# Quantus-Network/qp-zk-circuits

Hardware: AMD Instinct MI355X
Metric: Wormhole proofs/sec (higher is better)
Workload: dtype u64

## Files before the change

### include/qpgpu.h

```cpp
#ifndef QPGPU_H
#define QPGPU_H
#include <stddef.h>
#include <stdint.h>

#ifdef __cplusplus
extern "C" {
#endif

typedef struct qpgpu_ctx qpgpu_ctx;
typedef struct qpgpu_circuit qpgpu_circuit;

enum {
    QPGPU_OK = 0,
    QPGPU_EINVAL = -1,
    QPGPU_EDEVICE = -2,
    QPGPU_ENOMEM = -3,
    QPGPU_EUNSAT = -4,
    QPGPU_EBUFSIZE = -5
};

int qpgpu_ctx_create(int device, qpgpu_ctx **out);
void qpgpu_ctx_destroy(qpgpu_ctx *ctx);
const char *qpgpu_last_error(const qpgpu_ctx *ctx);
int qpgpu_ctx_set_stream(qpgpu_ctx *ctx, void *hip_stream);
// ... 20 lines not shown
int qpgpu_set_hasher(int kind, const uint64_t *params, size_t n_words);
int qpgpu_get_hasher(void);

enum {
    QPGPU_NTT_FORWARD = 0,
    QPGPU_NTT_INVERSE = 1,
    QPGPU_NTT_OUT_BITREV = 2
};
int qpgpu_ntt_batch(qpgpu_ctx *ctx, uint64_t *data, unsigned log_n, size_t batch, int flags,
                    uint64_t coset_shift);
int qpgpu_ntt_batch_dev(qpgpu_ctx *ctx, const uint64_t *d_in, uint64_t *d_out, unsigned log_n,
                        size_t batch, int flags, uint64_t coset_shift);
int qpgpu_lde_batch_dev(qpgpu_ctx *ctx, const uint64_t *d_coeffs, uint64_t *d_out, unsigned log_n,
                        unsigned rate_bits, size_t batch, int flags, uint64_t coset_shift);

int qpgpu_poseidon_permute_dev(qpgpu_ctx *ctx, uint64_t *d_states, size_t n);
int qpgpu_poseidon2_hash_pad10_dev(qpgpu_ctx *ctx, const uint64_t *params, size_t n_words, const uint64_t *d_in, size_t len,
                                   size_t count, uint64_t *d_out);
size_t qpgpu_merkle_digest_count(unsigned log_leaves, unsigned cap_height);
int qpgpu_merkle_build_dev(qpgpu_ctx *ctx, const uint64_t *d_cols, uint64_t col_stride, uint32_t n_cols,
                           unsigned log_leaves, unsigned cap_height, uint64_t *d_digests, uint64_t *h_cap_out);
int qpgpu_merkle_build_rows_dev(qpgpu_ctx *ctx, const uint64_t *d_rows, uint32_t width, unsigned log_leaves,
                                unsigned cap_height, uint64_t *d_digests, uint64_t *h_cap_out);

int qpgpu_circuit_load(qpgpu_ctx *ctx, const uint64_t *pack_words, size_t n_words, qpgpu_circuit **out);
int qpgpu_circuit_load_batch(qpgpu_ctx *ctx, const uint64_t *pack_words, size_t n_words, unsigned max_batch, qpgpu_circuit **out);
unsigned qpgpu_circuit_max_batch(const qpgpu_circuit *c);
size_t qpgpu_circuit_num_public_inputs(const qpgpu_circuit *c);
void qpgpu_circuit_free(qpgpu_circuit *c);
int qpgpu_circuit_scrub(qpgpu_circuit *c);
int qpgpu_circuit_constants_sigmas_cap(const qpgpu_circuit *c, uint64_t *out, size_t out_words);
int qpgpu_circuit_set_blinding_seed(qpgpu_circuit *c, uint64_t seed);
int qpgpu_circuit_set_witness_check(qpgpu_circuit *c, int on);
size_t qpgpu_proof_size(const qpgpu_circuit *c);
int qpgpu_prove(qpgpu_circuit *c, const uint64_t *wires, const uint64_t *public_inputs, uint8_t *out, size_t out_cap, size_t *out_len);
int qpgpu_prove_dev(qpgpu_circuit *c, const uint64_t *d_wires, const uint64_t *public_inputs, uint8_t *out, size_t out_cap, size_t *out_len);
int qpgpu_prove_batch_dev(qpgpu_circuit *c, const uint64_t *const *d_wires, uint32_t batch, const uint64_t *const *public_inputs,
                          uint8_t *const *outs, size_t out_cap, size_t *out_lens);

int qpgpu_witness_info(qpgpu_circuit *c, uint64_t *num_generators, uint64_t *num_levels, uint64_t *num_free_cells);
int qpgpu_witness_free_mask(qpgpu_circuit *c, uint8_t *mask, size_t mask_len);
int qpgpu_generate_witness_dev(qpgpu_circuit *c, uint64_t *d_wires, const uint64_t *public_inputs);
int qpgpu_generate_witness(qpgpu_circuit *c, uint64_t *wires, const uint64_t *public_inputs);
int qpgpu_circuit_gate_rows(const qpgpu_circuit *c, unsigned gate_type, uint32_t *rows_out, size_t cap, size_t *count);
int qpgpu_generate_witness_batch_dev(qpgpu_circuit *c, uint64_t *d_wires, uint32_t batch, const uint64_t *public_inputs);
int qpgpu_generate_witness_partial_dev(qpgpu_circuit *c, const uint64_t *cells, const uint64_t *values, size_t count,
                                       const uint64_t *public_inputs, uint64_t *d_wires);
int qpgpu_generate_witness_partial_batch_dev(qpgpu_circuit *c, const uint64_t *cells, size_t count, const uint64_t *values,
                                             const uint64_t *public_inputs, uint32_t batch, uint64_t *d_wires, int *status);
int qpgpu_witness_partial_prepare(qpgpu_circuit *c, const uint64_t *cells, size_t count, uint32_t max_batch);
int qpgpu_generate_witness_partial_batch_blinded_dev(qpgpu_circuit *c, const uint64_t *cells, size_t count, size_t n_blinding, const uint64_t *values,
                                                     const uint8_t *seeds, const uint64_t *public_inputs, uint32_t batch, uint64_t *d_wires, int *status);
int qpgpu_witness_public_inputs_dev(qpgpu_circuit *c, const uint64_t *d_wires, uint32_t batch, uint64_t *public_inputs_out);

typedef struct qpgpu_oracle qpgpu_oracle;
#define QPGPU_ORACLE_VALUES 0u
#define QPGPU_ORACLE_COEFFS 1u
#define QPGPU_ORACLE_BLINDING 2u
#define QPGPU_ORACLE_DEVICE_INPUT 4u
int qpgpu_oracle_commit(qpgpu_ctx *ctx, const uint64_t *polys, uint32_t num_polys, unsigned degree_bits, unsigned rate_bits,
                        unsigned cap_height, unsigned flags, uint64_t blinding_seed, uint32_t blinding_stream, qpgpu_oracle **out);
void qpgpu_oracle_free(qpgpu_oracle *o);
int qpgpu_oracle_cap(const qpgpu_oracle *o, uint64_t *out, size_t out_words);
int qpgpu_oracle_eval(qpgpu_oracle *o, const uint64_t point[2], uint32_t first, uint32_t count, uint64_t *out);
#define QPGPU_ORACLE_READ_COEFFS 0u
#define QPGPU_ORACLE_READ_LDE 1u
// ... 73 lines not shown
```

### qp-zk-circuits_amd/binding.py

```python
import ctypes
import os

import numpy as np

P = 0xFFFFFFFF00000001
MULT_GEN = 14293326489335486720

NTT_FORWARD = 0
NTT_INVERSE = 1
NTT_OUT_BITREV = 2

_HERE = os.path.dirname(os.path.abspath(__file__))


def lib_path():
    return os.path.join(_HERE, "libqpgpu.so")


class QpGpuError(RuntimeError):
    def __init__(self, code, msg):
        super().__init__(f"qpgpu error {code}: {msg}")
        self.code = code


# ... 44 lines not shown
        "qpgpu_zk_tree_build": (c.c_int, [vp, vp, c.c_size_t, c.c_uint, c.c_uint, c.POINTER(vp), c.c_char_p]),
        "qpgpu_zk_tree_free": (None, [vp]),
        "qpgpu_zk_tree_depth": (c.c_uint, [vp]),
        "qpgpu_zk_tree_leaf_count": (c.c_size_t, [vp]),
        "qpgpu_zk_tree_root": (c.c_int, [vp, vp]),
        "qpgpu_zk_tree_read_level": (c.c_int, [vp, c.c_uint, c.c_size_t, c.c_size_t, vp]),
        "qpgpu_zk_tree_open": (c.c_int, [vp, vp, c.c_size_t, vp, vp]),
        "qpgpu_zk_tree_build_reserved": (c.c_int, [vp, vp, c.c_size_t, c.c_size_t, c.c_uint, c.c_uint, c.POINTER(vp), c.c_char_p]),
        "qpgpu_zk_tree_capacity": (c.c_size_t, [vp]),
        "qpgpu_zk_tree_append": (c.c_int, [vp, vp, c.c_size_t, c.c_uint, vp, c.c_char_p]),
        "qpgpu_zk_tree_snapshot": (c.c_int, [vp, vp]),
        "qpgpu_zk_tree_open_at": (c.c_int, [vp, vp, vp, c.c_size_t, vp, vp]),
        "qpgpu_poseidon2_hash_pad10": (c.c_int, [u64p, c.c_size_t, u64p, c.c_size_t, u64p]),
        "qpgpu_crash_trace_armed": (c.c_int, []),
        "qpgpu_circuit_num_public_inputs": (c.c_size_t, [vp]),
        "qpgpu_merkle_digest_count": (c.c_size_t, [c.c_uint, c.c_uint]),
        "qpgpu_merkle_build_dev": (c.c_int, [vp, u64p, c.c_uint64, c.c_uint32, c.c_uint, c.c_uint, u64p, u64p]),
        "qpgpu_merkle_build_rows_dev": (c.c_int, [vp, u64p, c.c_uint32, c.c_uint, c.c_uint, u64p, u64p]),
        "qpgpu_circuit_load": (c.c_int, [vp, u64p, c.c_size_t, c.POINTER(vp)]),
        "qpgpu_circuit_load_batch": (c.c_int, [vp, u64p, c.c_size_t, c.c_uint, c.POINTER(vp)]),
        "qpgpu_circuit_max_batch": (c.c_uint, [vp]),
        "qpgpu_circuit_scrub": (c.c_int, [vp]),
        "qpgpu_prove_batch_dev": (c.c_int, [vp, vp, c.c_uint32, vp, vp, c.c_size_t, vp]),
        "qpgpu_ctx_set_hasher": (c.c_int, [vp, c.c_int, u64p, c.c_size_t]),
        "qpgpu_ctx_get_hasher": (c.c_int, [vp]),
        "qpgpu_ctx_challenger_observe": (c.c_int, [vp, vp, u64p, c.c_size_t]),
        "qpgpu_ctx_challenger_get": (c.c_int, [vp, vp, c.POINTER(c.c_uint64)]),
        "qpgpu_pool_create_batched": (c.c_int, [c.c_int, u64p, c.c_size_t, c.c_uint, c.c_uint, c.POINTER(vp)]),
        "qpgpu_circuit_free": (None, [vp]),
        "qpgpu_circuit_constants_sigmas_cap": (c.c_int, [vp, u64p, c.c_size_t]),
        "qpgpu_proof_size": (c.c_size_t, [vp]),
        "qpgpu_circuit_set_blinding_seed": (c.c_int, [vp, c.c_uint64]),
        "qpgpu_circuit_set_witness_check": (c.c_int, [vp, c.c_int]),
        "qpgpu_circuit_gate_rows": (c.c_int, [vp, c.c_uint, vp, c.c_size_t, c.POINTER(c.c_size_t)]),
        "qpgpu_prove": (c.c_int, [vp, u64p, u64p, vp, c.c_size_t, c.POINTER(c.c_size_t)]),
        "qpgpu_prove_dev": (c.c_int, [vp, u64p, u64p, vp, c.c_size_t, c.POINTER(c.c_size_t)]),
        "qpgpu_poseidon_constants": (c.c_size_t, [u64p, u64p, c.c_size_t]),
        "qpgpu_pool_create": (c.c_int, [c.c_int, u64p, c.c_size_t, c.c_uint, c.POINTER(vp)]),
        "qpgpu_pool_destroy": (None, [vp]),
        "qpgpu_pool_proof_size": (c.c_size_t, [vp]),
        "qpgpu_pool_workers": (c.c_uint, [vp]),
        "qpgpu_pool_last_error": (c.c_char_p, [vp]),
        "qpgpu_pool_submit": (c.c_int, [vp, u64p, u64p, vp, c.c_size_t, c.POINTER(c.c_uint64)]),
        "qpgpu_pool_wait": (c.c_int, [vp, c.c_uint64, c.POINTER(c.c_size_t)]),
        "qpgpu_pool_set_witness_check": (c.c_int, [vp, c.c_int]),
        "qpgpu_pool_create_multi": (c.c_int, [vp, c.c_uint, u64p, c.c_size_t, c.c_uint, c.c_uint, c.c_uint, c.POINTER(vp)]),
        "qpgpu_pool_devices": (c.c_uint, [vp]),
        "qpgpu_pool_serialized": (c.c_int, [vp]),
        "qpgpu_pool_set_partial_cells": (c.c_int, [vp, u64p, c.c_size_t]),
        "qpgpu_pool_set_partial_cells_blinded": (c.c_int, [vp, u64p, c.c_size_t, c.c_size_t]),
        "qpgpu_pool_submit_on": (c.c_int, [vp, c.c_uint, u64p, u64p, vp, c.c_size_t, c.POINTER(c.c_uint64)]),
        "qpgpu_pool_submit_host": (c.c_int, [vp, u64p, u64p, vp, c.c_size_t, c.POINTER(c.c_uint64)]),
        "qpgpu_pool_submit_partial": (c.c_int, [vp, u64p, u64p, vp, c.c_size_t, c.POINTER(c.c_uint64)]),
        "qpgpu_set_hasher": (c.c_int, [c.c_int, u64p, c.c_size_t]),
        "qpgpu_get_hasher": (c.c_int, []),
        "qpgpu_witness_info": (c.c_int, [vp, c.POINTER(c.c_uint64), c.POINTER(c.c_uint64), c.POINTER(c.c_uint64)]),
        "qpgpu_witness_free_mask": (c.c_int, [vp, vp, c.c_size_t]),
        "qpgpu_generate_witness_dev": (c.c_int, [vp, u64p, u64p]),
        "qpgpu_generate_witness": (c.c_int, [vp, u64p, u64p]),
        "qpgpu_generate_witness_batch_dev": (c.c_int, [vp, u64p, c.c_uint32, u64p]),
        "qpgpu_generate_witness_partial_dev": (c.c_int, [vp, u64p, u64p, c.c_size_t, u64p, u64p]),
        "qpgpu_generate_witness_partial_batch_dev": (c.c_int, [vp, u64p, c.c_size_t, u64p, u64p, c.c_uint32, u64p, vp]),
        "qpgpu_generate_witness_partial_batch_blinded_dev": (c.c_int, [vp, u64p, c.c_size_t, c.c_size_t, u64p, c.c_char_p, u64p, c.c_uint32, u64p, vp]),
        "qpgpu_witness_public_inputs_dev": (c.c_int, [vp, u64p, c.c_uint32, u64p]),
        "qpgpu_witness_partial_prepare": (c.c_int, [vp, u64p, c.c_size_t, c.c_uint32]),
        "qpgpu_oracle_commit": (c.c_int, [vp, u64p, c.c_uint32, c.c_uint, c.c_uint, c.c_uint, c.c_uint, c.c_uint64, c.c_uint32,
# ... 282 lines not shown
        h = ctypes.c_void_p()
        gpu._check(gpu.lib.qpgpu_circuit_load_batch(gpu.ctx, pw.ctypes.data, pw.size, max_batch, ctypes.byref(h)))
        self.h = h
        self.max_batch = max_batch
        self.num_public_inputs = int(pw[9])

    def scrub(self):
        self.gpu._check(self.gpu.lib.qpgpu_circuit_scrub(self.h))

    def prove_batch_dev(self, d_wires_list, public_inputs_list, outs=None):
        nb = len(d_wires_list)
        ptrs = (ctypes.c_void_p * nb)(*[_ptr(w) for w in d_wires_list])
        pis = [np.ascontiguousarray(p, dtype=np.uint64) for p in public_inputs_list]
        pip = (ctypes.c_void_p * nb)(*[p.ctypes.data for p in pis])
        size = self.proof_size()
        if outs is None:
            outs = [np.empty(size, dtype=np.uint8) for _ in range(nb)]
        op = (ctypes.c_void_p * nb)(*[o.ctypes.data for o in outs])
        lens = (ctypes.c_size_t * nb)()
        self.gpu._check(self.gpu.lib.qpgpu_prove_batch_dev(self.h, ptrs, nb, pip, op, size, lens))
        return [outs[i][:lens[i]].tobytes() for i in range(nb)]

    def close(self):
        if self.h:
            self.gpu.lib.qpgpu_circuit_free(self.h)
            self.h = None

    def proof_size(self):
        return self.gpu.lib.qpgpu_proof_size(self.h)

    def set_witness_check(self, on=True):
        self.gpu._check(self.gpu.lib.qpgpu_circuit_set_witness_check(self.h, 1 if on else 0))

    def set_blinding_seed(self, seed):
        self.gpu._check(self.gpu.lib.qpgpu_circuit_set_blinding_seed(self.h, seed))

    def constants_sigmas_cap(self, cap_height=4):
        out = np.empty((1 << cap_height, 4), dtype=np.uint64)
        self.gpu._check(self.gpu.lib.qpgpu_circuit_constants_sigmas_cap(self.h, out.ctypes.data, out.size))
        return out

    def witness_info(self):
        a, b, c3 = ctypes.c_uint64(), ctypes.c_uint64(), ctypes.c_uint64()
        self.gpu._check(self.gpu.lib.qpgpu_witness_info(self.h, ctypes.byref(a), ctypes.byref(b), ctypes.byref(c3)))
        return a.value, b.value, c3.value

    def gate_rows(self, gate_type):
        n = ctypes.c_size_t()
        self.gpu._check(self.gpu.lib.qpgpu_circuit_gate_rows(self.h, gate_type, None, 0, ctypes.byref(n)))
        rows = np.empty(n.value, dtype=np.uint32)
        self.gpu._check(self.gpu.lib.qpgpu_circuit_gate_rows(self.h, gate_type, rows.ctypes.data, rows.size, ctypes.byref(n)))
        return rows

    def witness_free_mask(self, num_wires, n):
        m = np.empty((num_wires, n), dtype=np.uint8)
        self.gpu._check(self.gpu.lib.qpgpu_witness_free_mask(self.h, m.ctypes.data, m.size))
        return m

    def generate_witness(self, wires, public_inputs):
        w = np.array(wires, dtype=np.uint64, order="C", copy=True)
        p = np.ascontiguousarray(public_inputs, dtype=np.uint64)
        self.gpu._check(self.gpu.lib.qpgpu_generate_witness(self.h, w.ctypes.data, p.ctypes.data))
        return w

    def generate_witness_dev(self, d_wires, public_inputs, batch=1):
        p = np.ascontiguousarray(public_inputs, dtype=np.uint64)
# ... 464 lines not shown
```

### qp-zk-circuits_amd/csrc/circuit_state.hpp

```cpp
#pragma once
#include <hip/hip_runtime.h>
#include <algorithm>
#include <vector>
#include "circuit.hpp"
#include "ctx.hpp"
#include "prover_host.hpp"
#include "prover_kernels.hpp"

struct WitnessPlan;
void witness_plan_free(WitnessPlan *p);

struct qpgpu_circuit {
    qpgpu_ctx *ctx = nullptr;
    CircuitPack pack;
    proof_layout::Proof layout;
    std::vector<void *> allocs;
    std::vector<std::pair<void *, size_t>> secret_allocs;
    uint32_t max_batch = 1;
    gl::u64 *d_cs_values = nullptr;
    PolyOracle cs;
    GateDev *d_gates = nullptr;
    std::vector<GateDev> h_gates;
    gl::u64 *d_qacc = nullptr;
    gl::u64 *d_poseidon_rc = nullptr, *d_poseidon_fast = nullptr;
    bool has_p2_gate = false;
    gl::u64 *d_omega = nullptr, *d_x_coset = nullptr, *d_l0_coset = nullptr, *d_zh_inv = nullptr;
    gl::u64 *d_ginv_lo = nullptr, *d_ginv_hi = nullptr; uint32_t ginv_lo_bits = 0;
    gl::u64 *d_wires_vals = nullptr;
    uint32_t *d_salt_keys = nullptr;
    PolyOracle wires, zs, quot;
    gl::u64 *d_qcp = nullptr, *d_rowprod = nullptr, *d_z = nullptr, *d_zs_vals = nullptr;
    gl::u64 *d_small = nullptr;
    size_t small_words = 0;
    gl::u64 *d_fold = nullptr;
    size_t fold_words = 0;
    gl::e2 *d_points = nullptr, *d_open = nullptr;
    FriParams fri;
    FriWork fri_work;
    Stager stage;
    bool seed_set = false;
    bool check_witness = false;
    gl::u64 *d_check = nullptr;
    gl::u64 blinding_seed = 0;
    WitnessPlan *wplan = nullptr;
    int witness_wide_rows = -1;

    template <class T> int alloc(T **p, size_t count, bool secret = false) {
        void *v = nullptr;
        const size_t bytes = std::max<size_t>(count * sizeof(T), 8);
        hipError_t e = hipMalloc(&v, bytes);
        if (e == hipErrorOutOfMemory) return ctx->fail(QPGPU_ENOMEM, "hipMalloc(circuit): out of device memory");
        if (e != hipSuccess) return ctx->hip_fail(e, "hipMalloc(circuit)");
        allocs.push_back(v);
        if (secret) secret_allocs.push_back({v, bytes});
        *p = (T *)v;
        return QPGPU_OK;
    }
};
```

### qp-zk-circuits_amd/csrc/prover.cpp

```cpp
#include <hip/hip_runtime.h>
#include <algorithm>
#include <array>
#include <cstring>
#include <random>
#include <string>
#include <vector>
#include "circuit.hpp"
#include "ctx.hpp"
#include "gl64.hpp"
#include "merkle.hpp"
#include "poseidon.hpp"
#include "prover_host.hpp"
#include "circuit_state.hpp"
#include "prover_kernels.hpp"

using gl::e2;
using gl::u64;

namespace {

std::vector<u64> powers_table(u64 base, u64 count) {
    std::vector<u64> t(count);
    u64 a = 1;
    for (u64 i = 0; i < count; i++) { t[i] = gl::canon(a); a = gl::mul(a, base); }
// ... 171 lines not shown
    CK(c->alloc(&c->d_zs_vals, (size_t)B * p.num_zs_pp_cols() * n, true));
    const size_t nterms = nch + nch * p.num_chunks() + p.num_gate_constraints;
    c->small_words = (2 * nch + nch * R + nch * nterms + 4 + 3) & ~(size_t)3;
    CK(c->alloc(&c->d_small, (size_t)B * c->small_words));
    {
        const uint32_t n_hash = pk_count_hash_gates(gd.data(), (uint32_t)gd.size());
        const char *e = getenv("QPGPU_QUOTIENT_FOLD");
        if (n_hash > 0 && n_hash <= qfold::MAX_GATES && !(e && *e == '0')) {
            c->fold_words = (size_t)n_hash * nch * qfold::WORDS;
            CK(c->alloc(&c->d_fold, (size_t)B * c->fold_words));
        }
    }
    const size_t n_open = p.num_cs_cols() + p.num_wires + p.num_zs_pp_cols() + p.num_quotient_cols();
    CK(c->alloc(&c->d_points, (size_t)B * 2));
    CK(c->alloc(&c->d_open, (size_t)B * (n_open + nch), true));
    {
        c->fri.degree_bits = d; c->fri.rate_bits = (unsigned)p.rate_bits; c->fri.cap_h = (unsigned)p.cap_height;
        c->fri.pow_bits = (unsigned)p.proof_of_work_bits; c->fri.num_queries = (uint32_t)p.num_query_rounds;
        for (u64 a : p.arity_bits) c->fri.arity_bits.push_back((unsigned)a);
        const std::vector<size_t> widths(c->layout.widths, c->layout.widths + 4);
        u64 *base = nullptr;
        CK(c->alloc(&base, FriWork::words(c->fri, widths, n_open, B), true));
        c->fri_work.bind(base, c->fri, widths, n_open, B);
        CK(c->alloc(&c->d_check, (size_t)B * 2));
    }
    {
        c->stage.words = (size_t)B * (c->small_words + 8 + 4 + 8) + FriWork::stage_words(c->fri, n_open, B) + 64;
        if (const char *e = getenv("QPGPU_STAGE_FALLBACK")) if (*e == '1') c->stage.words = 1;
        void *hp = nullptr;
        hipError_t e = hipHostMalloc(&hp, c->stage.words * 8, hipHostMallocDefault);
        if (e != hipSuccess) return fail(ctx->hip_fail(e, "hipHostMalloc(stage)"));
        c->stage.h = (u64 *)hp;
    }
    if (const char *e = getenv("QPGPU_WITNESS_WIDE_ROWS")) if (*e == '0' || *e == '1') c->witness_wide_rows = *e - '0';
    if ((rc = ctx->reserve_read_back((size_t)B * qpgpu_proof_size(c) + (1u << 16))) != QPGPU_OK) return fail(rc);
    CK(plan_transforms(c));
    {
        const hipError_t e = hipStreamSynchronize(ctx->stream);
        if (e != hipSuccess) return fail(ctx->hip_fail(e, "circuit_load: hipStreamSynchronize"));
    }
#undef CK
    *out = c;
    return QPGPU_OK;
}

int qpgpu_circuit_load(qpgpu_ctx *ctx, const uint64_t *pack_words, size_t n_words, qpgpu_circuit **out) {
    return qpgpu_circuit_load_batch(ctx, pack_words, n_words, 1, out);
}

unsigned qpgpu_circuit_max_batch(const qpgpu_circuit *c) { return c ? c->max_batch : 0; }
size_t qpgpu_circuit_num_public_inputs(const qpgpu_circuit *c) { return c ? (size_t)c->pack.num_public_inputs : 0; }

int qpgpu_circuit_set_witness_check(qpgpu_circuit *c, int on) {
    if (!c) return QPGPU_EINVAL;
    c->check_witness = on != 0;
    return QPGPU_OK;
}

int qpgpu_circuit_set_blinding_seed(qpgpu_circuit *c, uint64_t seed) {
    if (!c) return QPGPU_EINVAL;
    c->blinding_seed = seed; c->seed_set = true;
    return QPGPU_OK;
}

int qpgpu_circuit_constants_sigmas_cap(const qpgpu_circuit *c, uint64_t *out, size_t out_words) {
    if (!c || !out || out_words < c->cs.cap.size()) return QPGPU_EINVAL;
    std::memcpy(out, c->cs.cap.data(), c->cs.cap.size() * 8);
    return QPGPU_OK;
}

}

static int prove_batch_impl(qpgpu_circuit *c, uint32_t nb, const u64 *d_wires, const u64 *const *public_inputs, uint8_t *const *outs, size_t out_cap, size_t *out_lens) {
    qpgpu_ctx *ctx = c->ctx;
    const CircuitPack &p = c->pack;
    hipStream_t st = ctx->stream;
    const u64 n = p.n(), lde_n = n << p.rate_bits, R = p.num_routed_wires;
    const uint32_t nch = (uint32_t)p.num_challenges, npp = (uint32_t)p.num_partial_products, nchunks = npp + 1;
    const unsigned d = (unsigned)p.degree_bits, L = (unsigned)(p.degree_bits + p.rate_bits), cap_h = (unsigned)p.cap_height;
    const size_t ncs = p.num_cs_cols(), NW = p.num_wires, nzp = p.num_zs_pp_cols(), nq = p.num_quotient_cols();
    const size_t sig0 = p.num_selectors + p.num_constants, cap_words = (1ull << cap_h) * 4;
    const size_t nterms = nch + nch * nchunks + p.num_gate_constraints;
    unsigned qbits = 0; while ((1ull << qbits) < p.quotient_degree_factor) qbits++;
    const unsigned Lq = d + qbits, q_shift = (unsigned)p.rate_bits - qbits;
    const u64 q_n = 1ull << Lq;
    const size_t SW = c->small_words;

    c->stage.pos = 0;
// ... 73 lines not shown
    QP_HIP(ctx, pk_quotient_fold_sweep(qa, c->h_gates.data(), st));
    if (c->check_witness) {
        QuotientArgs ta{};
        ta.wires = d_wires; ta.cs = c->d_cs_values; ta.alpha_pows = d_apow; ta.pi_hash = d_pih; ta.gates = c->d_gates;
        ta.acc = c->d_qacc; ta.out = c->d_qacc; ta.poseidon_rc = c->d_poseidon_rc;
        ta.p2_gate = ctx->d_p2_app; ta.p2_layout = p.p2_layout;
        ta.zh_inv = c->d_zh_inv; ta.lde_n = n; ta.q_n = n; ta.q_shift = 0; ta.log_lde = d; ta.rate = 1; ta.nch = nch; ta.num_routed = (uint32_t)R;
        ta.chunk = (uint32_t)p.quotient_degree_factor; ta.nchunks = nchunks; ta.sig0 = (uint32_t)sig0;
        ta.num_selectors = (uint32_t)p.num_selectors; ta.num_gates = (uint32_t)p.gates.size(); ta.nterms = (uint32_t)nterms;
        ta.batch = nb; ta.ps_wires = NW * n; ta.ps_zs = 0; ta.ps_small = SW; ta.ps_acc = (u64)nch * n; ta.ps_out = (u64)nch * n;
        ta.fold = c->d_fold; ta.ps_fold = c->fold_words;
        QP_HIP(ctx, hipMemsetAsync(c->d_qacc, 0, (size_t)nb * nch * n * 8, st));
        std::vector<u64> init(2 * (size_t)nb);
        for (uint32_t b = 0; b < nb; b++) { init[2 * b] = ~0ull; init[2 * b + 1] = 0; }
        QP_TRY(c->stage.put(ctx, c->d_check, init.data(), init.size() * 8));
        QP_HIP(ctx, pk_gate_sums(ta, c->h_gates.data(), st));
        QP_HIP(ctx, pk_witness_check(c->d_qacc, n, nch, c->d_z, c->d_rowprod, c->d_check, nb, st));
        std::vector<u64> res(2 * (size_t)nb);
        QP_TRY(ctx->read_back(res.data(), c->d_check, res.size() * 8));
        for (uint32_t b = 0; b < nb; b++) {
            const std::string who = nb > 1 ? " (proof " + std::to_string(b) + " of the batch)" : "";
            if (res[2 * b] != ~0ull) return ctx->fail(QPGPU_EUNSAT, "witness does not satisfy the circuit: gate constraints fail at row " + std::to_string(res[2 * b]) + who);
            if (res[2 * b + 1]) return ctx->fail(QPGPU_EUNSAT, "witness does not satisfy the circuit: a copy constraint is violated (permutation product != 1)" + who);
        }
    }
    ctx->prof_begin("prove_quotient");
    qa.wires = c->wires.lde; qa.cs = c->cs.lde; qa.zs_pp = c->zs.lde; qa.x_coset = c->d_x_coset; qa.l0_coset = c->d_l0_coset;
    qa.zh_inv = c->d_zh_inv; qa.alpha_pows = d_apow; qa.beta_k_is = d_bk; qa.betas = d_betas; qa.gammas = d_gammas; qa.pi_hash = d_pih;
    qa.gates = c->d_gates; qa.acc = c->d_qacc; qa.poseidon_rc = c->d_poseidon_rc; qa.out = c->quot.coeffs;
    qa.p2_gate = ctx->d_p2_app; qa.p2_layout = p.p2_layout; qa.lde_n = lde_n; qa.q_n = q_n; qa.q_shift = q_shift; qa.log_lde = L; qa.rate = 1u << p.rate_bits; qa.nch = nch;
    qa.num_routed = (uint32_t)R; qa.chunk = (uint32_t)p.quotient_degree_factor; qa.nchunks = nchunks; qa.sig0 = (uint32_t)sig0;
    qa.num_selectors = (uint32_t)p.num_selectors; qa.num_gates = (uint32_t)p.gates.size(); qa.nterms = (uint32_t)nterms;
    qa.batch = nb; qa.ps_wires = c->wires.ps_lde; qa.ps_zs = c->zs.ps_lde; qa.ps_small = SW; qa.ps_acc = (u64)nch * lde_n; qa.ps_out = (u64)nch * q_n;
    QP_HIP(ctx, pk_quotient(qa, c->h_gates.data(), st));
    QP_TRY(ntt_run(ctx, c->quot.coeffs, c->quot.coeffs, Lq, Lq, (size_t)nch * nb, true, false, 0));
    QP_HIP(ctx, pk_scale_powers(c->quot.coeffs, q_n, (u64)nch * nb, c->d_ginv_lo, c->d_ginv_hi, c->ginv_lo_bits, st));
    ctx->prof_end();
    ctx->prof_begin("prove_commit_quotient");
    QP_TRY(oracle_commit_coeffs(ctx, c->quot, c->d_salt_keys));
    ctx->prof_end();
    std::vector<e2> zetas(nb), g_zetas(nb), pts(2 * (size_t)nb);
    for (uint32_t b = 0; b < nb; b++) {
        Challenger &ch = chs[b];
        ch.observe(c->quot.cap_of(b), cap_words);
        const e2 zeta = ch.get_ext();
        {
            e2 zn = zeta;
            for (unsigned i = 0; i < d; i++) zn = gl::e2_mul(zn, zn);
            zn = gl::e2_canon(zn);
            if (zn.a == 1 && zn.b == 0) return ctx->fail(QPGPU_EINVAL, "prove: opening point is in the subgroup");
        }
        zetas[b] = zeta;
        g_zetas[b] = gl::e2_canon(gl::e2_scale(zeta, gl::root_of_unity(d)));
        pts[2 * b] = zeta; pts[2 * b + 1] = g_zetas[b];
    }

    ctx->prof_begin("prove_openings");
    const size_t n_open = ncs + NW + nzp + nq, OW = n_open + nch;
    {
        QP_TRY(c->stage.put(ctx, c->d_points, pts.data(), pts.size() * sizeof(e2)));
        const PolyOracle *bs[4] = {&c->cs, &c->wires, &c->zs, &c->quot};
        size_t off = 0;
        for (const PolyOracle *o : bs) { QP_HIP(ctx, pk_poly_eval(o->coeffs, n, o->ncols, c->d_points, 1, c->d_open + off, nb, o->ps_coeffs, 2, OW, st)); off += o->ncols; }
        QP_HIP(ctx, pk_poly_eval(c->zs.coeffs, n, nch, c->d_points + 1, 1, c->d_open + n_open, nb, c->zs.ps_coeffs, 2, OW, st));
    }
    std::vector<e2> open((size_t)nb * OW);
// ... 85 lines not shown
```

### qp-zk-circuits_amd/csrc/quotient_kernels.hip

```cpp
#include <hip/hip_runtime.h>
#include "gl64.hpp"
#include "poseidon.hpp"
#include "quotient_kernels.hpp"

using gl::e2;
using gl::u32;
using gl::u64;

namespace {

__device__ __forceinline__ u64 gate_filter(const QuotientArgs &a, u32 gi, u64 s) {
    const GateDev g = a.gates[gi];
    u64 f = 1;
    for (u32 j = g.group_start; j < g.group_end; j++)
        if (j != gi) f = gl::mul(f, gl::sub((u64)j, s));
    if (a.num_selectors > 1) f = gl::mul(f, gl::sub(0xFFFFFFFFull, s));
    return f;
}


__device__ __forceinline__ void quotient_select_proof(QuotientArgs &a) {
    const u64 pr = blockIdx.z;
    a.wires += pr * a.ps_wires; a.zs_pp += pr * a.ps_zs;
    a.alpha_pows += pr * a.ps_small; a.beta_k_is += pr * a.ps_small; a.betas += pr * a.ps_small; a.gammas += pr * a.ps_small; a.pi_hash += pr * a.ps_small;
    a.acc += pr * a.ps_acc; a.out += pr * a.ps_out;
    if (a.fold) a.fold += pr * a.ps_fold;
}

template <int NCH>
__device__ __forceinline__ void quotient_add_store(const QuotientArgs &a, u64 S, u64 j, u64 f, const u64 (&sum)[NCH], int finalize) {
    if (finalize) {
        const u64 i = brev32((u32)j, a.log_lde);
        const u64 zi = a.zh_inv[i & (a.rate - 1)];
#pragma unroll
        for (int c = 0; c < NCH; c++) a.out[(u64)c * a.q_n + (i >> a.q_shift)] = gl::canon(gl::mul(gl::add(a.acc[(u64)c * S + j], gl::mul(f, sum[c])), zi));
    } else {
// ... 237 lines not shown
            for (; q & 7; ) {
                const u64 limb = w[(u64)--q * S];
                s2 = gl::add(gl::add(s2, s2), limb);
                emit(1 + q, gl::mul(limb, gl::sub(limb, 1)));
            }
#pragma unroll 1
            while (q) {
                q -= 8;
                u64 v[8];
#pragma unroll
                for (int i = 0; i < 8; i++) v[i] = w[(u64)(q + i) * S];
#pragma unroll
                for (int i = 7; i >= 0; i--) {
                    s2 = gl::add(gl::add(s2, s2), v[i]);
                    emit(1 + q + i, gl::mul(v[i], gl::sub(v[i], 1)));
                }
            }
            emit(0, gl::sub(s2, a.wires[j]));
        }
#pragma unroll
        for (int c = 0; c < NCH; c++) acc[c] = gl::add(acc[c], gl::mul(f, gl::acc_reduce(sum[c])));
    }
    if (finalize) {
        const u64 i = brev32((u32)j, a.log_lde);
        const u64 zi = a.zh_inv[i & (a.rate - 1)];
#pragma unroll
        for (int c = 0; c < NCH; c++) a.out[(u64)c * a.q_n + (i >> a.q_shift)] = gl::canon(gl::mul(acc[c], zi));
    } else {
#pragma unroll
        for (int c = 0; c < NCH; c++) a.acc[(u64)c * S + j] = acc[c];
    }
}

template <int NCH, u32 KIND>
__global__ void __launch_bounds__(256) quotient_hash_rounds_kernel(QuotientArgs a, qfold::Schedule s, u32 gi, u32 t0, int finalize) {
    const u64 j = blockIdx.x * (u64)blockDim.x + threadIdx.x;
    if (j >= a.q_n) return;
    s.kind = KIND;
    quotient_select_proof(a);
    const u64 S = a.lde_n;
    const u64 *ap = a.alpha_pows + t0;
    gl::Acc192 wsum[NCH];
#pragma unroll
    for (int c = 0; c < NCH; c++) wsum[c] = gl::acc_zero();
    qfold::walk(s, qfold::Consts{a.poseidon_rc, a.p2_gate}, WireAt{a.wires, S, j}, WeighInto<NCH>{wsum, ap, a.nterms});
    const u64 f = gate_filter(a, gi, a.cs[(u64)a.gates[gi].selector_index * S + j]);
    u64 sum[NCH];
#pragma unroll
    for (int c = 0; c < NCH; c++) sum[c] = gl::acc_reduce(wsum[c]);
    quotient_add_store(a, S, j, f, sum, finalize);
}

template <int N>
__device__ __forceinline__ void sbox7_group(u64 (&x)[N]) {
#if defined(__HIP_DEVICE_COMPILE__)
    u64 x2[N], x3[N], x4[N];
    gl::mul_group(x2, x, x);
    gl::mul_group(x4, x2, x2);
    gl::mul_group(x3, x, x2);
    gl::mul_group(x, x3, x4);
#else
    for (int i = 0; i < N; i++) x[i] = poseidon::sbox7(x[i]);
#endif
}
#ifndef FOLD_GROUP
#define FOLD_GROUP 4
// ... 109 lines not shown
    for (u32 i = 0; i < num_gates; i++) if (is_hash_gate(host_gates[i])) n++;
    return n;
}
static qfold::Schedule hash_gate_schedule(const QuotientArgs &a, const GateDev &g) {
    return g.type == GATE_POSEIDON ? qfold::poseidon_schedule() : qfold::poseidon2_schedule(a.p2_layout);
}
template <int NCH>
static void hash_gate_launch(const QuotientArgs &a, const GateDev *host_gates, u32 gi, u32 t0, u32 slot, int finalize, dim3 g, dim3 b, hipStream_t st) {
    const bool p1 = host_gates[gi].type == GATE_POSEIDON;
    const qfold::Schedule s = hash_gate_schedule(a, host_gates[gi]);
    if (a.fold) {
        if (p1) hipLaunchKernelGGL((quotient_poseidon_kernel<NCH>), g, b, 0, st, a, s, gi, t0, slot, finalize);
        else hipLaunchKernelGGL((quotient_poseidon2_kernel<NCH>), g, b, 0, st, a, s, gi, t0, slot, finalize);
    } else {
        if (p1) hipLaunchKernelGGL((quotient_hash_rounds_kernel<NCH, GATE_POSEIDON>), g, b, 0, st, a, s, gi, t0, finalize);
        else hipLaunchKernelGGL((quotient_hash_rounds_kernel<NCH, GATE_POSEIDON2>), g, b, 0, st, a, s, gi, t0, finalize);
    }
}
hipError_t pk_quotient_fold_sweep(const QuotientArgs &a, const GateDev *host_gates, hipStream_t st) {
    if (!a.fold || a.batch == 0) return hipSuccess;
    FoldSweepArgs fa{};
    for (u32 i = 0; i < a.num_gates; i++)
        if (is_hash_gate(host_gates[i])) {
            if (fa.ngates == qfold::MAX_GATES) return hipErrorInvalidValue;
            fa.sched[fa.ngates++] = hash_gate_schedule(a, host_gates[i]);
        }
    if (fa.ngates == 0) return hipSuccess;
    fa.nch = a.nch; fa.nterms = a.nterms; fa.t0 = a.nch + a.nch * a.nchunks; fa.batch = a.batch;
    fa.alpha_pows = a.alpha_pows; fa.poseidon_rc = a.poseidon_rc; fa.p2_gate = a.p2_gate;
    fa.fold = const_cast<u64 *>(a.fold); fa.ps_small = a.ps_small; fa.ps_fold = a.ps_fold;
    hipLaunchKernelGGL(quotient_fold_sweep_kernel, dim3(fa.ngates, fa.nch, fa.batch), dim3(64), 0, st, fa);
    return hipGetLastError();
}
template <int NCH>
static hipError_t quotient_launch(const QuotientArgs &a, const GateDev *host_gates, bool perm, bool finalize, hipStream_t st) {
    dim3 b(256), g((unsigned)((a.q_n + 255) / 256), 1, a.batch);
    const u32 t0 = a.nch + a.nch * a.nchunks;
    const u32 n_hash = pk_count_hash_gates(host_gates, a.num_gates);
    if (perm) hipLaunchKernelGGL((quotient_perm_kernel<NCH>), g, b, 0, st, a);
    const int fin_gates = finalize && n_hash == 0;
    if (wide_random_access(a, host_gates)) hipLaunchKernelGGL((quotient_gates_kernel<NCH, true>), g, b, 0, st, a, t0, fin_gates);
    else hipLaunchKernelGGL((quotient_gates_kernel<NCH, false>), g, b, 0, st, a, t0, fin_gates);
    u32 slot = 0;
    for (u32 i = 0; i < a.num_gates; i++)
        if (is_hash_gate(host_gates[i])) {
            hash_gate_launch<NCH>(a, host_gates, i, t0, slot, finalize && slot + 1 == n_hash, g, b, st);
            slot++;
        }
    return hipGetLastError();
}
static hipError_t quotient_dispatch(const QuotientArgs &a, const GateDev *host_gates, bool perm, bool finalize, hipStream_t st) {
    switch (a.nch) {
        case 1: return quotient_launch<1>(a, host_gates, perm, finalize, st);
        case 2: return quotient_launch<2>(a, host_gates, perm, finalize, st);
        case 3: return quotient_launch<3>(a, host_gates, perm, finalize, st);
        case 4: return quotient_launch<4>(a, host_gates, perm, finalize, st);
        default: return hipErrorInvalidValue;
    }
}
hipError_t pk_quotient(const QuotientArgs &a, const GateDev *host_gates, hipStream_t st) {
    if (a.q_n == 0 || a.batch == 0) return hipSuccess;
    return quotient_dispatch(a, host_gates, true, true, st);
}
hipError_t pk_gate_sums(const QuotientArgs &a, const GateDev *host_gates, hipStream_t st) { return quotient_dispatch(a, host_gates, false, false, st); }
hipError_t pk_witness_check(const u64 *acc, u64 n, u32 nch, const u64 *z, const u64 *rowprod, u64 *result, u32 batch, hipStream_t st) {
    if (n > 0 && batch > 0) hipLaunchKernelGGL(witness_check_kernel, dim3((unsigned)((n + 255) / 256), 1, batch), dim3(256), 0, st, acc, n, nch, z, rowprod, result);
    return hipGetLastError();
}
```

### qp-zk-circuits_amd/csrc/quotient_kernels.hpp

```cpp
#pragma once
#include <hip/hip_runtime.h>
#include <stdint.h>
#include "circuit.hpp"
#include "gl64.hpp"
#include "quotient_fold.hpp"

struct GateDev { uint32_t type, param0, param1, selector_index, group_start, group_end, num_constraints, param2; };

struct QuotientArgs {
    const uint64_t *wires, *cs, *zs_pp;
    const uint64_t *x_coset, *l0_coset;
    const uint64_t *zh_inv;
    const uint64_t *alpha_pows;
    const uint64_t *beta_k_is, *betas, *gammas, *pi_hash;
    const GateDev *gates;
    const uint64_t *poseidon_rc;
    const poseidon2::Params *p2_gate;
    P2GateLayout p2_layout;
    uint64_t *acc;
    uint64_t *out;
    uint64_t lde_n;
    uint64_t q_n;
    uint32_t q_shift;
    uint32_t log_lde, rate, nch, num_routed, chunk, nchunks, sig0, num_selectors, num_gates, nterms;
    uint32_t batch;
    uint64_t ps_wires, ps_zs, ps_small, ps_acc, ps_out;
    const uint64_t *fold;
    uint64_t ps_fold;
};

struct FoldSweepArgs {
    qfold::Schedule sched[qfold::MAX_GATES];
    uint32_t ngates, nch, nterms, t0, batch;
    const uint64_t *alpha_pows;
    const uint64_t *poseidon_rc;
    const poseidon2::Params *p2_gate;
    uint64_t *fold;
    uint64_t ps_small, ps_fold;
};

hipError_t pk_quotient(const QuotientArgs &a, const GateDev *host_gates, hipStream_t st);
uint32_t pk_count_hash_gates(const GateDev *host_gates, uint32_t num_gates);
hipError_t pk_quotient_fold_sweep(const QuotientArgs &a, const GateDev *host_gates, hipStream_t st);
hipError_t pk_gate_sums(const QuotientArgs &a, const GateDev *host_gates, hipStream_t st);
hipError_t pk_witness_check(const uint64_t *acc, uint64_t n, uint32_t nch, const uint64_t *z, const uint64_t *rowprod, uint64_t *result, uint32_t batch, hipStream_t st);

__device__ __forceinline__ uint32_t brev32(uint32_t x, uint32_t bits) { return bits ? __brev(x) >> (32 - bits) : 0; }
```

Measured before the change: 1468.

## Fuse quotient permutation and non-hash gate evaluation into one XCD-aware kernel

Adds a fused quotient kernel that evaluates the permutation argument and the constant, public-input, arithmetic and base-sum gate constraints in a single pass over chunks of routed wires. Each wire and sigma column is read once instead of separately by the perm and gates kernels. It also adds a 1D grid mapping that groups tiles across the 8 XCDs and interleaves proofs, aimed at better L2 locality. It is on by default when the circuit's gate set fits the fused pattern, with env and API switches to disable it. The cost is higher register pressure from the accumulator arrays.

```diff
diff --git a/include/qpgpu.h b/include/qpgpu.h
--- a/include/qpgpu.h
+++ b/include/qpgpu.h
@@ -76,6 +76,8 @@
 int qpgpu_circuit_constants_sigmas_cap(const qpgpu_circuit *c, uint64_t *out, size_t out_words);
 int qpgpu_circuit_set_blinding_seed(qpgpu_circuit *c, uint64_t seed);
 int qpgpu_circuit_set_witness_check(qpgpu_circuit *c, int on);
+int qpgpu_circuit_set_quotient_fused(qpgpu_circuit *c, int on);
+int qpgpu_circuit_quotient_info(const qpgpu_circuit *c, int *fused_enabled, int *fused_selected);
 size_t qpgpu_proof_size(const qpgpu_circuit *c);
 int qpgpu_prove(qpgpu_circuit *c, const uint64_t *wires, const uint64_t *public_inputs, uint8_t *out, size_t out_cap, size_t *out_len);
 int qpgpu_prove_dev(qpgpu_circuit *c, const uint64_t *d_wires, const uint64_t *public_inputs, uint8_t *out, size_t out_cap, size_t *out_len);
diff --git a/qp-zk-circuits_amd/binding.py b/qp-zk-circuits_amd/binding.py
--- a/qp-zk-circuits_amd/binding.py
+++ b/qp-zk-circuits_amd/binding.py
@@ -100,6 +100,8 @@
         "qpgpu_proof_size": (c.c_size_t, [vp]),
         "qpgpu_circuit_set_blinding_seed": (c.c_int, [vp, c.c_uint64]),
         "qpgpu_circuit_set_witness_check": (c.c_int, [vp, c.c_int]),
+        "qpgpu_circuit_set_quotient_fused": (c.c_int, [vp, c.c_int]),
+        "qpgpu_circuit_quotient_info": (c.c_int, [vp, c.POINTER(c.c_int), c.POINTER(c.c_int)]),
         "qpgpu_circuit_gate_rows": (c.c_int, [vp, c.c_uint, vp, c.c_size_t, c.POINTER(c.c_size_t)]),
         "qpgpu_prove": (c.c_int, [vp, u64p, u64p, vp, c.c_size_t, c.POINTER(c.c_size_t)]),
         "qpgpu_prove_dev": (c.c_int, [vp, u64p, u64p, vp, c.c_size_t, c.POINTER(c.c_size_t)]),
@@ -448,6 +450,14 @@
     def set_witness_check(self, on=True):
         self.gpu._check(self.gpu.lib.qpgpu_circuit_set_witness_check(self.h, 1 if on else 0))
 
+    def set_quotient_fused(self, on=True):
+        self.gpu._check(self.gpu.lib.qpgpu_circuit_set_quotient_fused(self.h, 1 if on else 0))
+
+    def quotient_info(self):
+        a, b = ctypes.c_int(), ctypes.c_int()
+        self.gpu._check(self.gpu.lib.qpgpu_circuit_quotient_info(self.h, ctypes.byref(a), ctypes.byref(b)))
+        return bool(a.value), bool(b.value)
+
     def set_blinding_seed(self, seed):
         self.gpu._check(self.gpu.lib.qpgpu_circuit_set_blinding_seed(self.h, seed))
 
diff --git a/qp-zk-circuits_amd/csrc/circuit_state.hpp b/qp-zk-circuits_amd/csrc/circuit_state.hpp
--- a/qp-zk-circuits_amd/csrc/circuit_state.hpp
+++ b/qp-zk-circuits_amd/csrc/circuit_state.hpp
@@ -40,6 +40,8 @@
     Stager stage;
     bool seed_set = false;
     bool check_witness = false;
+    bool quotient_fused = true;
+    bool quotient_plain_map = false;
     gl::u64 *d_check = nullptr;
     gl::u64 blinding_seed = 0;
     WitnessPlan *wplan = nullptr;
diff --git a/qp-zk-circuits_amd/csrc/prover.cpp b/qp-zk-circuits_amd/csrc/prover.cpp
--- a/qp-zk-circuits_amd/csrc/prover.cpp
+++ b/qp-zk-circuits_amd/csrc/prover.cpp
@@ -227,6 +227,8 @@
         if (e != hipSuccess) return fail(ctx->hip_fail(e, "hipHostMalloc(stage)"));
         c->stage.h = (u64 *)hp;
     }
+    if (const char *e = getenv("QPGPU_QUOTIENT_FUSED")) if (*e == '0') c->quotient_fused = false;
+    if (const char *e = getenv("QPGPU_QUOTIENT_XCD_MAP")) if (*e == '0') c->quotient_plain_map = true;
     if (const char *e = getenv("QPGPU_WITNESS_WIDE_ROWS")) if (*e == '0' || *e == '1') c->witness_wide_rows = *e - '0';
     if ((rc = ctx->reserve_read_back((size_t)B * qpgpu_proof_size(c) + (1u << 16))) != QPGPU_OK) return fail(rc);
     CK(plan_transforms(c));
@@ -249,6 +251,22 @@
 int qpgpu_circuit_set_witness_check(qpgpu_circuit *c, int on) {
     if (!c) return QPGPU_EINVAL;
     c->check_witness = on != 0;
+    return QPGPU_OK;
+}
+
+int qpgpu_circuit_set_quotient_fused(qpgpu_circuit *c, int on) {
+    if (!c) return QPGPU_EINVAL;
+    c->quotient_fused = on != 0;
+    return QPGPU_OK;
+}
+
+int qpgpu_circuit_quotient_info(const qpgpu_circuit *c, int *fused_enabled, int *fused_selected) {
+    if (!c) return QPGPU_EINVAL;
+    const CircuitPack &p = c->pack;
+    const bool fits = pk_quotient_fused_gates(c->h_gates.data(), (uint32_t)c->h_gates.size(), (uint32_t)p.num_routed_wires,
+                                              (uint32_t)p.quotient_degree_factor, (uint32_t)p.num_partial_products + 1, nullptr);
+    if (fused_enabled) *fused_enabled = c->quotient_fused ? 1 : 0;
+    if (fused_selected) *fused_selected = c->quotient_fused && fits ? 1 : 0;
     return QPGPU_OK;
 }
 
@@ -388,6 +406,7 @@
     qa.num_routed = (uint32_t)R; qa.chunk = (uint32_t)p.quotient_degree_factor; qa.nchunks = nchunks; qa.sig0 = (uint32_t)sig0;
     qa.num_selectors = (uint32_t)p.num_selectors; qa.num_gates = (uint32_t)p.gates.size(); qa.nterms = (uint32_t)nterms;
     qa.batch = nb; qa.ps_wires = c->wires.ps_lde; qa.ps_zs = c->zs.ps_lde; qa.ps_small = SW; qa.ps_acc = (u64)nch * lde_n; qa.ps_out = (u64)nch * q_n;
+    qa.fused = c->quotient_fused ? 1 : 0; qa.fused_plain_map = c->quotient_plain_map ? 1 : 0;
     QP_HIP(ctx, pk_quotient(qa, c->h_gates.data(), st));
     QP_TRY(ntt_run(ctx, c->quot.coeffs, c->quot.coeffs, Lq, Lq, (size_t)nch * nb, true, false, 0));
     QP_HIP(ctx, pk_scale_powers(c->quot.coeffs, q_n, (u64)nch * nb, c->d_ginv_lo, c->d_ginv_hi, c->ginv_lo_bits, st));
diff --git a/qp-zk-circuits_amd/csrc/quotient_kernels.hip b/qp-zk-circuits_amd/csrc/quotient_kernels.hip
--- a/qp-zk-circuits_amd/csrc/quotient_kernels.hip
+++ b/qp-zk-circuits_amd/csrc/quotient_kernels.hip
@@ -2,6 +2,7 @@
 #include "gl64.hpp"
 #include "poseidon.hpp"
 #include "quotient_kernels.hpp"
+#include "quotient_map.hpp"
 
 using gl::e2;
 using gl::u32;
@@ -305,6 +306,147 @@
     }
 }
 
+constexpr u32 FUSED_CHUNK = 8;
+constexpr u32 FUSED_NONE = 0xFFFFFFFFu;
+
+template <int NCH>
+__global__ void __launch_bounds__(256, NCH <= 2 ? 4 : 2) quotient_perm_gates_kernel(QuotientArgs a, FusedGates fg, u32 tiles, u32 grouped, int finalize) {
+    const qmap::Place pl = qmap::place(blockIdx.x, tiles, a.batch, grouped != 0);
+    if (!pl.valid) return;
+    const u64 j = pl.tile * (u64)blockDim.x + threadIdx.x;
+    if (j >= a.q_n) return;
+    {
+        const u64 pr = pl.proof;
+        a.wires += pr * a.ps_wires; a.zs_pp += pr * a.ps_zs;
+        a.alpha_pows += pr * a.ps_small; a.beta_k_is += pr * a.ps_small; a.betas += pr * a.ps_small; a.gammas += pr * a.ps_small; a.pi_hash += pr * a.ps_small;
+        a.acc += pr * a.ps_acc; a.out += pr * a.ps_out;
+    }
+    const u32 logL = a.log_lde, R = a.num_routed, nchunks = a.nchunks, npp = nchunks - 1;
+    const u64 i = brev32((u32)j, logL);
+    const u64 jn = brev32((u32)((i + a.rate) & (a.lde_n - 1)), logL);
+    const u64 x = a.x_coset[j], S = a.lde_n;
+    const u64 *consts_base = a.cs + (u64)a.num_selectors * S + j;
+    const u64 *gp = a.alpha_pows + NCH + NCH * nchunks;
+    const u32 n_ops = fg.n_ops, n_limbs = fg.n_limbs;
+    gl::Acc192 acc[NCH], asum[NCH], bsum[NCH];
+#pragma unroll
+    for (int c = 0; c < NCH; c++) { acc[c] = gl::acc_zero(); asum[c] = gl::acc_zero(); bsum[c] = gl::acc_zero(); }
+    u64 nxt[NCH];
+    {
+        const u64 l0 = a.l0_coset[j];
+#pragma unroll
+        for (int k = 0; k < NCH; k++) {
+            const u64 term = gl::mul(l0, gl::sub(a.zs_pp[(u64)k * S + j], 1));
+#pragma unroll
+            for (int c = 0; c < NCH; c++) gl::acc_mul(acc[c], term, a.alpha_pows[(u64)c * a.nterms + k]);
+            nxt[k] = a.zs_pp[(u64)k * S + jn];
+        }
+    }
+    u64 s2 = 0;
+    u64 gsum[NCH];
+#pragma unroll
+    for (int c = 0; c < NCH; c++) gsum[c] = 0;
+    auto fold_gate = [&](u32 gi, const gl::Acc192 (&sum)[NCH]) {
+        const u64 f = gate_filter(a, gi, a.cs[(u64)a.gates[gi].selector_index * S + j]);
+#pragma unroll
+        for (int c = 0; c < NCH; c++) gsum[c] = gl::add(gsum[c], gl::mul(f, gl::acc_reduce(sum[c])));
+    };
+    auto wire = [&](u32 r, u64 v, u64 sg, u64 (&pn)[NCH], u64 (&pd)[NCH]) {
+#pragma unroll
+        for (int k = 0; k < NCH; k++) {
+            const u64 sid = gl::mul(a.beta_k_is[k * R + r], x);
+            const u64 ssg = gl::mul(a.betas[k], sg);
+            pn[k] = gl::mul(pn[k], gl::add(gl::add(v, sid), a.gammas[k]));
+            pd[k] = gl::mul(pd[k], gl::add(gl::add(v, ssg), a.gammas[k]));
+        }
+        const bool limb = r >= 1 && r <= n_limbs;
+        const u64 twice = gl::add(gl::add(s2, s2), v), cst = gl::mul(v, gl::sub(v, 1));
+        s2 = limb ? twice : s2;
+#pragma unroll
+        for (int c = 0; c < NCH; c++) { const u64 wt = gp[(u64)c * a.nterms + (limb ? r : 0)]; gl::acc_mul(bsum[c], cst, limb ? wt : 0); }
+    };
+    auto arith = [&](u32 q, u64 m0, u64 m1, u64 ad, u64 out, u64 c0, u64 c1) {
+        const bool op = q < n_ops;
+        const u64 cst = gl::sub(out, gl::add(gl::mul(gl::mul(m0, m1), c0), gl::mul(ad, c1)));
+#pragma unroll
+        for (int c = 0; c < NCH; c++) { const u64 wt = gp[(u64)c * a.nterms + (op ? q : 0)]; gl::acc_mul(asum[c], cst, op ? wt : 0); }
+    };
+#pragma unroll 1
+    for (u32 cc = nchunks; cc-- > 0; ) {
+        const u32 r0 = cc * FUSED_CHUNK, m = R - r0 < FUSED_CHUNK ? R - r0 : FUSED_CHUNK;
+        u64 w[FUSED_CHUNK], pn[NCH], pd[NCH], prv[NCH];
+#pragma unroll
+        for (int k = 0; k < NCH; k++) { pn[k] = 1; pd[k] = 1; prv[k] = cc == 0 ? a.zs_pp[(u64)k * S + j] : a.zs_pp[((u64)NCH + (u64)k * npp + cc - 1) * S + j]; }
+        const u64 c0 = consts_base[0], c1 = consts_base[S];
+        if (m == FUSED_CHUNK) {
+            u64 sg[FUSED_CHUNK];
+#pragma unroll
+            for (u32 t = 0; t < FUSED_CHUNK; t++) { w[t] = a.wires[(u64)(r0 + t) * S + j]; sg[t] = a.cs[(u64)(a.sig0 + r0 + t) * S + j]; }
+#pragma unroll
+            for (int t = FUSED_CHUNK - 1; t >= 0; t--) {
+                wire(r0 + t, w[t], sg[t], pn, pd);
+                if (t % 4 == 0) arith((r0 + t) / 4, w[t], w[t + 1], w[t + 2], w[t + 3], c0, c1);
+            }
+        } else {
+#pragma unroll
+            for (int t = FUSED_CHUNK - 1; t >= 0; t--) {
+                w[t] = 0;
+                if ((u32)t < m) { w[t] = a.wires[(u64)(r0 + t) * S + j]; wire(r0 + t, w[t], a.cs[(u64)(a.sig0 + r0 + t) * S + j], pn, pd); }
+                if (t % 4 == 0 && (r0 + t) / 4 < n_ops) arith((r0 + t) / 4, w[t], w[t + 1], w[t + 2], w[t + 3], c0, c1);
+            }
+        }
+#pragma unroll
+        for (int k = 0; k < NCH; k++) {
+            const u64 term = gl::sub(gl::mul(prv[k], pn[k]), gl::mul(nxt[k], pd[k]));
+#pragma unroll
+            for (int c = 0; c < NCH; c++) gl::acc_mul(acc[c], term, a.alpha_pows[(u64)c * a.nterms + NCH + k * nchunks + cc]);
+            nxt[k] = prv[k];
+        }
+        if (cc == 0) {
+            if (fg.base_sum != FUSED_NONE) {
+                const u64 cst = gl::sub(s2, w[0]);
+#pragma unroll
+                for (int c = 0; c < NCH; c++) gl::acc_mul(bsum[c], cst, gp[(u64)c * a.nterms]);
+                fold_gate(fg.base_sum, bsum);
+            }
+            if (fg.arithmetic != FUSED_NONE) fold_gate(fg.arithmetic, asum);
+            if (fg.constant != FUSED_NONE) {
+                gl::Acc192 sum[NCH];
+#pragma unroll
+                for (int c = 0; c < NCH; c++) sum[c] = gl::acc_zero();
+#pragma unroll
+                for (u32 q = 0; q < 4; q++)
+                    if (q < fg.n_consts) {
+                        const u64 cst = gl::sub(consts_base[(u64)q * S], w[q]);
+#pragma unroll
+                        for (int c = 0; c < NCH; c++) gl::acc_mul(sum[c], cst, gp[(u64)c * a.nterms + q]);
+                    }
+                fold_gate(fg.constant, sum);
+            }
+            if (fg.public_input != FUSED_NONE) {
+                gl::Acc192 sum[NCH];
+#pragma unroll
+                for (int c = 0; c < NCH; c++) sum[c] = gl::acc_zero();
+#pragma unroll
+                for (u32 q = 0; q < 4; q++) {
+                    const u64 cst = gl::sub(w[q], a.pi_hash[q]);
+#pragma unroll
+                    for (int c = 0; c < NCH; c++) gl::acc_mul(sum[c], cst, gp[(u64)c * a.nterms + q]);
+                }
+                fold_gate(fg.public_input, sum);
+            }
+        }
+    }
+    if (finalize) {
+        const u64 zi = a.zh_inv[i & (a.rate - 1)];
+#pragma unroll
+        for (int c = 0; c < NCH; c++) a.out[(u64)c * a.q_n + (i >> a.q_shift)] = gl::canon(gl::mul(gl::add(gl::acc_reduce(acc[c]), gsum[c]), zi));
+    } else {
+#pragma unroll
+        for (int c = 0; c < NCH; c++) a.acc[(u64)c * S + j] = gl::add(gl::acc_reduce(acc[c]), gsum[c]);
+    }
+}
+
 template <int NCH, u32 KIND>
 __global__ void __launch_bounds__(256) quotient_hash_rounds_kernel(QuotientArgs a, qfold::Schedule s, u32 gi, u32 t0, int finalize) {
     const u64 j = blockIdx.x * (u64)blockDim.x + threadIdx.x;
@@ -480,15 +622,38 @@
     hipLaunchKernelGGL(quotient_fold_sweep_kernel, dim3(fa.ngates, fa.nch, fa.batch), dim3(64), 0, st, fa);
     return hipGetLastError();
 }
+bool pk_quotient_fused_gates(const GateDev *host_gates, uint32_t num_gates, uint32_t num_routed, uint32_t chunk, uint32_t nchunks, FusedGates *out) {
+    FusedGates fg{FUSED_NONE, FUSED_NONE, FUSED_NONE, FUSED_NONE, 0, 0, 0};
+    if (chunk != FUSED_CHUNK || num_routed < FUSED_CHUNK || nchunks != (num_routed + FUSED_CHUNK - 1) / FUSED_CHUNK) return false;
+    for (u32 i = 0; i < num_gates; i++) {
+        const GateDev &g = host_gates[i];
+        if (g.num_constraints == 0 || g.type == GATE_POSEIDON || g.type == GATE_POSEIDON2) continue;
+        if (g.type == GATE_CONSTANT && fg.constant == FUSED_NONE && g.param0 <= 4) { fg.constant = i; fg.n_consts = g.param0; }
+        else if (g.type == GATE_PUBLIC_INPUT && fg.public_input == FUSED_NONE) fg.public_input = i;
+        else if (g.type == GATE_ARITHMETIC && fg.arithmetic == FUSED_NONE && g.param0 >= 1 && (uint64_t)4 * g.param0 <= num_routed) { fg.arithmetic = i; fg.n_ops = g.param0; }
+        else if (g.type == GATE_BASE_SUM && fg.base_sum == FUSED_NONE && g.param0 >= 1 && (uint64_t)g.param0 + 1 <= num_routed) { fg.base_sum = i; fg.n_limbs = g.param0; }
+        else return false;
+    }
+    if (out) *out = fg;
+    return true;
+}
 template <int NCH>
 static hipError_t quotient_launch(const QuotientArgs &a, const GateDev *host_gates, bool perm, bool finalize, hipStream_t st) {
     dim3 b(256), g((unsigned)((a.q_n + 255) / 256), 1, a.batch);
     const u32 t0 = a.nch + a.nch * a.nchunks;
     const u32 n_hash = pk_count_hash_gates(host_gates, a.num_gates);
-    if (perm) hipLaunchKernelGGL((quotient_perm_kernel<NCH>), g, b, 0, st, a);
     const int fin_gates = finalize && n_hash == 0;
-    if (wide_random_access(a, host_gates)) hipLaunchKernelGGL((quotient_gates_kernel<NCH, true>), g, b, 0, st, a, t0, fin_gates);
-    else hipLaunchKernelGGL((quotient_gates_kernel<NCH, false>), g, b, 0, st, a, t0, fin_gates);
+    FusedGates fg;
+    const u32 tiles = g.x;
+    const bool grouped = a.fused_plain_map == 0;
+    if (perm && a.fused && pk_quotient_fused_gates(host_gates, a.num_gates, a.num_routed, a.chunk, a.nchunks, &fg) &&
+        qmap::grid_size(tiles, a.batch, grouped) <= 0x7FFFFFFFull) {
+        hipLaunchKernelGGL((quotient_perm_gates_kernel<NCH>), dim3((unsigned)qmap::grid_size(tiles, a.batch, grouped)), b, 0, st, a, fg, tiles, grouped ? 1u : 0u, fin_gates);
+    } else {
+        if (perm) hipLaunchKernelGGL((quotient_perm_kernel<NCH>), g, b, 0, st, a);
+        if (wide_random_access(a, host_gates)) hipLaunchKernelGGL((quotient_gates_kernel<NCH, true>), g, b, 0, st, a, t0, fin_gates);
+        else hipLaunchKernelGGL((quotient_gates_kernel<NCH, false>), g, b, 0, st, a, t0, fin_gates);
+    }
     u32 slot = 0;
     for (u32 i = 0; i < a.num_gates; i++)
         if (is_hash_gate(host_gates[i])) {
diff --git a/qp-zk-circuits_amd/csrc/quotient_kernels.hpp b/qp-zk-circuits_amd/csrc/quotient_kernels.hpp
--- a/qp-zk-circuits_amd/csrc/quotient_kernels.hpp
+++ b/qp-zk-circuits_amd/csrc/quotient_kernels.hpp
@@ -27,7 +27,10 @@
     uint64_t ps_wires, ps_zs, ps_small, ps_acc, ps_out;
     const uint64_t *fold;
     uint64_t ps_fold;
+    uint32_t fused, fused_plain_map;
 };
+
+struct FusedGates { uint32_t constant, public_input, arithmetic, base_sum, n_consts, n_ops, n_limbs; };
 
 struct FoldSweepArgs {
     qfold::Schedule sched[qfold::MAX_GATES];
@@ -40,6 +43,7 @@
 };
 
 hipError_t pk_quotient(const QuotientArgs &a, const GateDev *host_gates, hipStream_t st);
+bool pk_quotient_fused_gates(const GateDev *host_gates, uint32_t num_gates, uint32_t num_routed, uint32_t chunk, uint32_t nchunks, FusedGates *out);
 uint32_t pk_count_hash_gates(const GateDev *host_gates, uint32_t num_gates);
 hipError_t pk_quotient_fold_sweep(const QuotientArgs &a, const GateDev *host_gates, hipStream_t st);
 hipError_t pk_gate_sums(const QuotientArgs &a, const GateDev *host_gates, hipStream_t st);
diff --git a/qp-zk-circuits_amd/csrc/quotient_map.hpp b/qp-zk-circuits_amd/csrc/quotient_map.hpp
--- /dev/null
+++ b/qp-zk-circuits_amd/csrc/quotient_map.hpp
@@ -0,0 +1,33 @@
+#pragma once
+#include <stdint.h>
+
+#if defined(__HIPCC__)
+#define QMAP_HD __host__ __device__ __forceinline__
+#else
+#define QMAP_HD inline
+#endif
+
+namespace qmap {
+
+constexpr uint32_t XCDS = 8;
+
+struct Place { uint32_t tile, proof; bool valid; };
+
+QMAP_HD uint64_t grid_size(uint32_t tiles, uint32_t batch, bool grouped) {
+    return grouped ? (uint64_t)((tiles + XCDS - 1) / XCDS) * XCDS * batch : (uint64_t)tiles * batch;
+}
+QMAP_HD Place place(uint32_t id, uint32_t tiles, uint32_t batch, bool grouped) {
+    Place p;
+    if (grouped) {
+        const uint32_t per_group = XCDS * batch, w = id % per_group;
+        p.tile = XCDS * (id / per_group) + w % XCDS;
+        p.proof = w / XCDS;
+    } else {
+        p.tile = id % tiles;
+        p.proof = id / tiles;
+    }
+    p.valid = p.tile < tiles && p.proof < batch;
+    return p;
+}
+
+}
```

New measurement: 1495, median of 6. 1.02x the previous value.
